# AI-Application-and-Integration-Lab/RDPN6D

Measured on AMD Instinct MI355X. Metric: RGB-D crops/sec (fwd+PnP) at 256x256, higher is better.
Workload: dtype f32

## Files before the change

### include/rdpn6d.h

```cpp
#ifndef RDPN6D_H
#define RDPN6D_H

#ifdef __cplusplus
extern "C" {
#endif

#define RDPN6D_OK 0
#define RDPN6D_EINVAL -1
#define RDPN6D_EHIP -2
#define RDPN6D_ENOMEM -3

const char* rdpn6d_last_error(void);
int rdpn6d_version(void);
int rdpn6d_device_count(void);

void farthest_point_sampling(float* pts, int* idxs, int pn, int sn);
void farthest_point_sampling_init_center(float* pts, int* idxs, int pn, int sn);
int rdpn6d_fps_host(const float* pts, int* idxs, int pn, int sn, int start);
int rdpn6d_fps_device(const float* d_pts, const int* d_offsets, int nobj, int max_pn, int sn, int start,
                      int* d_idxs, float* d_mindist, void* stream);
long long rdpn6d_fps_workspace_bytes(int nobj);
int rdpn6d_fps_device_ws(const float* d_pts, const int* d_offsets, int nobj, int max_pn, int sn, int start, int* d_idxs,
                         float* d_mindist, void* workspace, long long workspace_bytes, void* stream);

// ... 9 lines not shown
    int in_cs, in_co;
    int Ho, Wo;
    int stride;
    int ntaps;
    int dy[9], dx[9];
    int N, Npad;
    int OH, OW;
    int osy, osx, ooy, oox;
    int out_cs, out_co;
    int res_cs, res_co;
    int act;
    float slope;
} rdpn6d_conv_desc;
int rdpn6d_conv2d_f32(const rdpn6d_conv_desc* d, void* stream);
long long rdpn6d_conv_splitk_ws_floats(const rdpn6d_conv_desc* d, int ksplit);
int rdpn6d_conv2d_splitk_f32(const rdpn6d_conv_desc* d, int ksplit, float* workspace, void* stream);
int rdpn6d_conv_tile_for(const rdpn6d_conv_desc* d, int* bm, int* bn);
void rdpn6d_conv_force_tile(int bm, int bn);
void rdpn6d_conv_set_tap_inner(int v);

int rdpn6d_conv2d_bf16(const rdpn6d_conv_desc* d, int out_f32, void* stream);
int rdpn6d_conv2d_splitk_bf16(const rdpn6d_conv_desc* d, int out_f32, int ksplit, float* workspace, void* stream);
int rdpn6d_conv2d_bf16_bnstats(const rdpn6d_conv_desc* d, double* stats, int stats_row0, int* stats_rows, void* stream);
int rdpn6d_conv2d_bf16_bnbwd(const rdpn6d_conv_desc* d, const void* bn_x, int bn_cs, int bn_co, const float* mean, const float* invstd,
                             const float* gamma, const float* beta, double* partial, int* rows, void* stream);
int rdpn6d_bn_relu_backward_apply_bf16(const void* x, int xcs, int xco, const void* dy, int dcs, int dco, const float* mean,
                                       const float* invstd, const float* gamma, const float* beta, float* dgamma, float* dbeta, void* dx,
                                       int xgcs, int xgco, long long M, int C, const double* partial, int S, void* stream);
int rdpn6d_conv2d_bf16_bnbwd_y(const rdpn6d_conv_desc* d, const void* bn_x, int bn_cs, int bn_co, const void* bn_y, int y_cs, int y_co,
                               const float* mean, const float* invstd, double* partial, int* rows, void* stream);
int rdpn6d_bn_backward_apply_bf16(const void* x, int xcs, int xco, const void* dy, int dcs, int dco, const void* y, int ycs, int yco,
                                  const float* mean, const float* invstd, const float* gamma, float* dgamma, float* dbeta, void* dx,
                                  int xgcs, int xgco, void* dres, int rcs, int rco, long long M, int C, const double* partial, int S,
                                  void* stream);
void rdpn6d_conv_bf16_force_tile(int bm, int bn);
void rdpn6d_conv_bf16_force_stages(int nst);
int rdpn6d_conv_bf16_tile_for(const rdpn6d_conv_desc* d, int* bm, int* bn);
int rdpn6d_conv_bf16_uses_pingpong(const rdpn6d_conv_desc* d, int out_f32);
int rdpn6d_split_bf16x3(const float* x, long long n, void* planes, long long plane_elems, void* stream);
int rdpn6d_conv_bf16x3_eligible(const rdpn6d_conv_desc* d);
int rdpn6d_conv_bf16x3_kernel_for(const rdpn6d_conv_desc* d);
int rdpn6d_conv2d_bf16x3(const rdpn6d_conv_desc* d, long long x_plane_elems, long long w_plane_elems, void* y_planes,
                         long long y_plane_elems, void* stream);
int rdpn6d_conv2d_bf16x3_ex(const rdpn6d_conv_desc* d, long long x_plane_elems, long long w_plane_elems, void* y_planes,
                            long long y_plane_elems, const void* res_planes, long long res_plane_elems, void* stream);
int rdpn6d_split_h2(const float* x, int src_cs, int src_co, int C, void* dst, long long npix, int* overflow_flag, void* stream);
int rdpn6d_conv_h2_kernel_for(const rdpn6d_conv_desc* d);
int rdpn6d_conv2d_h2(const rdpn6d_conv_desc* d, void* y_h2, const void* res_h2, int* overflow_flag, void* stream);
int rdpn6d_conv2d_h2_cb(const rdpn6d_conv_desc* d, void* y_h2, const void* res_h2, int* overflow_flag, const float* crop_bias,
                        void* stream);
long long rdpn6d_conv_h2_workspace_bytes(const rdpn6d_conv_desc* d);
void rdpn6d_conv_h2_set_clock_probe(unsigned long long* buf);
void rdpn6d_conv_h2_set_wfrag(int mode);
int rdpn6d_conv_h2_colmax_ok(const rdpn6d_conv_desc* d, int rows_per_group);
int rdpn6d_conv2d_h2_colmax(const rdpn6d_conv_desc* d, unsigned long long* keys, int rows_per_group, int* overflow_flag, void* stream);
int rdpn6d_h2_colmax_decode(unsigned long long* keys, int groups, int N, int Npad, void* out_h2, void* stream);
int rdpn6d_conv_h2_wfrag_wanted(const rdpn6d_conv_desc* d);
int rdpn6d_h2_weight_frag(const void* w_h2, int Npad, int ntaps, int cchunks, void* w_frag, void* stream);
int rdpn6d_conv2d_h2_wf(const rdpn6d_conv_desc* d, void* y_h2, const void* res_h2, int* overflow_flag, const void* w_frag, void* stream);
int rdpn6d_conv2d_h2_ws(const rdpn6d_conv_desc* d, void* y_h2, const void* res_h2, int* overflow_flag, const float* crop_bias,
                        void* workspace, long long workspace_bytes, void* stream);
int rdpn6d_conv_h2_fuse1x1_ok(const rdpn6d_conv_desc* d);
int rdpn6d_conv2d_h2_fuse1x1(const rdpn6d_conv_desc* d, const void* res_h2, int* overflow_flag, const float* crop_bias,
                             const void* w1_h2, const float* scale1, const float* bias1, float* out, int out_cs, int n_out,
                             void* stream);
int rdpn6d_upsample_bilinear_h2(const void* x, int B, int H, int W, int C, int factor, void* y, int* overflow_flag, void* stream);
int rdpn6d_upsample_bilinear_h2_ex(const void* x, int B, int H, int W, int C, int factor, void* y, int out_cs, int out_co, int relu,
                                   int* overflow_flag, void* stream);
int rdpn6d_xyz_subsample_h2(const float* x, int B, int xc, int R, int step, void* y, int out_cs, int out_co, int* overflow_flag,
                            void* stream);
int rdpn6d_global_max_concat_h2(void* buf, int B, int HW, int C, int cs, void* stream);
int rdpn6d_global_max_h2(const void* x_h2, int B, int HW, int C, int cs, void* gmax_h2, void* stream);
int rdpn6d_convt3x3s2_const_bias_f32(const float* V, const float* scale, int B, int F, float* out , void* stream);
int rdpn6d_stem_pool_h2(const float* x, int B, int xc, int R, const void* w_h2, const float* scale, const float* shift, void* y,
                        int* overflow_flag, void* stream);
int rdpn6d_stem_pool_h2_ex(const float* x, int B, int xc, int R, const void* w_h2, const float* scale, const float* shift, void* y,
                           int out_fmt, int* overflow_flag, void* stream);
int rdpn6d_stem_pack_h2(const float* w_oihw, void* w_h2, float* inv_scale, void* stream);
void rdpn6d_conv_bf16_force_chunk(int row_bytes);
int rdpn6d_stem_conv7x7_bf16(const float* x, int B, int xc, int R, const float* w, const float* scale,
                             const float* shift, void* y, void* stream);
int rdpn6d_maxpool3x3s2_bf16(const void* x, int B, int H, int W, int C, void* y, void* stream);
int rdpn6d_upsample_bilinear_bf16(const void* x, int B, int H, int W, int C, int factor, void* y, void* stream);
int rdpn6d_xyz_subsample_bf16(const float* x, int B, int xc, int R, int step, void* y, int out_cs, int out_co,
                              void* stream);
int rdpn6d_global_max_concat_bf16(void* buf, int B, int HW, int C, int cs, void* stream);
int rdpn6d_cast_f32_bf16(const float* src, int src_cs, int src_co, int C, void* dst, int dst_cs, long long npix,
                         void* stream);

int rdpn6d_stem_conv7x7_f32(const float* x, int B, int xc, int R, const float* w, const float* scale,
                            const float* shift, float* y, void* stream);
int rdpn6d_maxpool3x3s2_f32(const float* x, int B, int H, int W, int C, float* y, void* stream);
int rdpn6d_upsample_bilinear_f32(const float* x, int B, int H, int W, int C, int factor, float* y, void* stream);
int rdpn6d_xyz_subsample_f32(const float* x, int B, int xc, int R, int step, float* y, int out_cs, int out_co,
                             void* stream);
int rdpn6d_global_max_concat_f32(float* buf, int B, int HW, int C, int cs, void* stream);
int rdpn6d_groupnorm_relu_f32(float* x, int B, int HW, int C, int G, const float* gamma, const float* beta,
                              void* stream);
int rdpn6d_groupnorm_relu_h2(const float* x, int B, int HW, int C, int G, const float* gamma, const float* beta, void* y_h2,
                             int* overflow_flag, void* stream);

int rdpn6d_dense_glue_f32(const float* head, int head_cs, const float* coord2d, const float* fps, int B, int HW,
                          int K, int mask_attention, float* minmax_scratch, float* out_nchw, float* pnp_in,
                          int pnp_cs, int* argmax_out, void* stream);
int rdpn6d_dense_glue_h2(const float* head, int head_cs, const float* coord2d, const float* fps, int B, int HW, int K,
                         int mask_attention, float* minmax_scratch, float* out_nchw, void* pnp_in_h2, int pnp_cs,
// ... 260 lines not shown
```

### rdpn6d_amd/_lib.py

```python
import ctypes
import os

HERE = os.path.dirname(os.path.abspath(__file__))
LIB_PATH = os.environ.get("RDPN6D_LIB") or os.path.join(HERE, "librdpn6d_hip.so")

_ll = ctypes.c_longlong
c_float_p = ctypes.c_void_p
c_int_p = ctypes.c_void_p
_vp, _i, _f, _u = ctypes.c_void_p, ctypes.c_int, ctypes.c_float, ctypes.c_uint


class ConvDesc(ctypes.Structure):

    _fields_ = [
        ("x", _vp), ("w", _vp), ("scale", _vp), ("shift", _vp), ("res", _vp), ("y", _vp),
        ("B", _i), ("H", _i), ("W", _i), ("Cin", _i), ("in_cs", _i), ("in_co", _i), ("Ho", _i), ("Wo", _i),
        ("stride", _i), ("ntaps", _i), ("dy", _i * 9), ("dx", _i * 9), ("N", _i), ("Npad", _i), ("OH", _i), ("OW", _i),
        ("osy", _i), ("osx", _i), ("ooy", _i), ("oox", _i), ("out_cs", _i), ("out_co", _i), ("res_cs", _i),
        ("res_co", _i), ("act", _i), ("slope", _f),
    ]


SIGNATURES = {
    "rdpn6d_last_error": (ctypes.c_char_p, []),
# ... 83 lines not shown
    "rdpn6d_dense_glue_backward_f32": (_i, [_vp, _i, _vp, _vp, _vp, _vp, _i, _i, _i, _i, _i, _vp, _vp, _vp, _vp]),
    "rdpn6d_dense_losses_mt_f32": (_i, [_vp, _i, _vp, _vp, _vp, _vp, _i, _i, _i, _f, _f, _f, _i, _vp, _vp, _vp, _vp]),
    "rdpn6d_dense_glue_backward_mt_f32": (_i, [_vp, _i, _vp, _vp, _vp, _vp, _i, _i, _i, _i, _i, _i, _vp, _vp, _vp, _vp]),
    "rdpn6d_pose_train_f32": (_i, [_vp, _i, _vp, _vp, _vp, _vp, _vp, _vp, _vp, _vp, _i, _i, _i, _f, _i, _f, _f, _vp, _vp, _vp,
                                   _vp, _vp, _vp]),
    "rdpn6d_pose_train_sym_f32": (_i, [_vp, _i, _vp, _vp, _vp, _vp, _vp, _vp, _vp, _vp, _i, _i, _i, _f, _i, _f, _f, _vp, _vp, _i,
                                       _vp, _vp, _vp, _vp, _vp, _vp, _vp]),
    "rdpn6d_ranger_step_f32": (_i, [_vp, _vp, _vp, _vp, _vp, _vp, _i, _vp, _vp, _i, _vp, _f, _f, _f, _f, _f, _i, _i, _f, _vp]),
    "rdpn6d_ranger_step_scaled_f32": (_i, [_vp, _vp, _vp, _vp, _vp, _vp, _i, _vp, _vp, _i, _vp, _f, _f, _f, _f, _f, _i, _i, _f, _f, _vp, _vp]),
    "rdpn6d_grad_nonfinite_f32": (_i, [_vp, _ll, _vp, _vp]),
    "rdpn6d_region_targets_f32": (_i, [_vp, _vp, _vp, _vp, _i, _i, _i, _vp, _vp, _vp]),
    "rdpn6d_pose_errors_f64": (_i, [_vp, _vp, _vp, _i, _i, _i, _vp, _vp, _vp]),
    "rdpn6d_crop_builder_f32": (_i, [_vp, _vp, _i, _i, _i, _vp, _vp, _vp, _vp, _vp, _i, _i, _vp, _vp, _vp]),
    "rdpn6d_act_backward_f32": (_i, [_vp, _vp, _ll, _f, _vp]),
    "rdpn6d_transpose_rc_f32": (_i, [_vp, _i, _i, _i, _vp, _vp]),
    "rdpn6d_train_vis_scalars_f32": (_i, [_vp, _vp, _vp, _vp, _vp, _i, _vp, _i, _vp, _vp]),
    "rdpn6d_rgb_to_nhwc4_f32": (_i, [_vp, _i, _i, _i, _vp, _vp]),
    "rdpn6d_stem_im2col_f32": (_i, [_vp, _i, _i, _i, _vp, _vp]),
    "rdpn6d_stem_rowpatch_f32": (_i, [_vp, _i, _i, _i, _vp, _vp]),
    "rdpn6d_stem_conv7x7_raw_bf16": (_i, [_vp, _i, _i, _i, _vp, _vp, _vp]),
    "rdpn6d_bn_train_stats_bf16": (_i, [_vp, _ll, _i, _i, _i, _f, _f, _vp, _vp, _vp, _vp, _vp, _vp]),
    "rdpn6d_bn_apply_bf16": (_i, [_vp, _i, _i, _vp, _vp, _vp, _vp, _vp, _i, _i, _vp, _i, _i, _ll, _i, _i, _vp]),
    "rdpn6d_bn_backward_bf16": (_i, [_vp, _i, _i, _vp, _i, _i, _vp, _i, _i, _vp, _vp, _vp, _vp, _vp, _vp, _i, _i, _vp, _i, _i,
                                     _ll, _i, _i, _vp, _vp]),
    "rdpn6d_bn_relu_backward_bf16": (_i, [_vp, _i, _i, _vp, _i, _i, _vp, _vp, _vp, _vp, _vp, _vp, _vp, _i, _i, _ll, _i, _vp, _vp]),
    "rdpn6d_channel_sum_bf16": (_i, [_vp, _ll, _i, _i, _i, _vp, _i, _vp, _vp]),
    "rdpn6d_maxpool3x3s2_backward_bf16": (_i, [_vp, _vp, _i, _i, _i, _i, _vp, _vp]),
    "rdpn6d_upsample_bilinear_backward_bf16": (_i, [_vp, _i, _i, _i, _i, _i, _vp, _vp]),
    "rdpn6d_global_max_concat_backward_bf16": (_i, [_vp, _vp, _i, _i, _i, _i, _vp, _vp]),
    "rdpn6d_stem_im2col_bf16": (_i, [_vp, _i, _i, _i, _vp, _vp]),
    "rdpn6d_stem_rowpatch_bf16": (_i, [_vp, _i, _i, _i, _vp, _vp]),
    "rdpn6d_repack_f32": (_i, [_vp, _vp, _vp, _i, _vp]),
    "rdpn6d_split_h2": (_i, [_vp, _i, _i, _i, _vp, _ll, _vp, _vp]),
    "rdpn6d_conv_h2_kernel_for": (_i, [_vp]),
    "rdpn6d_conv2d_h2": (_i, [_vp, _vp, _vp, _vp, _vp]),
    "rdpn6d_upsample_bilinear_h2": (_i, [_vp, _i, _i, _i, _i, _i, _vp, _vp, _vp]),
    "rdpn6d_xyz_subsample_h2": (_i, [_vp, _i, _i, _i, _i, _vp, _i, _i, _vp, _vp]),
    "rdpn6d_stem_pool_h2": (_i, [_vp, _i, _i, _i, _vp, _vp, _vp, _vp, _vp, _vp]),
    "rdpn6d_stem_pool_h2_ex": (_i, [_vp, _i, _i, _i, _vp, _vp, _vp, _vp, _i, _vp, _vp]),
    "rdpn6d_stem_pack_h2": (_i, [_vp, _vp, _vp, _vp]),
    "rdpn6d_global_max_concat_h2": (_i, [_vp, _i, _i, _i, _i, _vp]),
    "rdpn6d_upsample_bilinear_h2_ex": (_i, [_vp, _i, _i, _i, _i, _i, _vp, _i, _i, _i, _vp, _vp]),
    "rdpn6d_global_max_h2": (_i, [_vp, _i, _i, _i, _i, _vp, _vp]),
    "rdpn6d_convt3x3s2_const_bias_f32": (_i, [_vp, _vp, _i, _i, _vp, _vp]),
    "rdpn6d_conv2d_h2_cb": (_i, [_vp, _vp, _vp, _vp, _vp, _vp]),
    "rdpn6d_conv2d_h2_ws": (_i, [_vp, _vp, _vp, _vp, _vp, _vp, ctypes.c_longlong, _vp]),
    "rdpn6d_conv_h2_fuse1x1_ok": (_i, [ctypes.POINTER(ConvDesc)]),
    "rdpn6d_conv2d_h2_fuse1x1": (_i, [ctypes.POINTER(ConvDesc), _vp, _vp, _vp, _vp, _vp, _vp, _vp, _i, _i, _vp]),
    "rdpn6d_conv_h2_workspace_bytes": (ctypes.c_longlong, [_vp]),
    "rdpn6d_conv_h2_colmax_ok": (_i, [ctypes.POINTER(ConvDesc), _i]),
    "rdpn6d_conv2d_h2_colmax": (_i, [ctypes.POINTER(ConvDesc), _vp, _i, _vp, _vp]),
    "rdpn6d_h2_colmax_decode": (_i, [_vp, _i, _i, _i, _vp, _vp]),
    "rdpn6d_conv_h2_set_wfrag": (None, [_i]),
    "rdpn6d_conv_h2_set_clock_probe": (None, [_vp]),
    "rdpn6d_conv_h2_wfrag_wanted": (_i, [ctypes.POINTER(ConvDesc)]),
    "rdpn6d_h2_weight_frag": (_i, [_vp, _i, _i, _i, _vp, _vp]),
    "rdpn6d_conv2d_h2_wf": (_i, [ctypes.POINTER(ConvDesc), _vp, _vp, _vp, _vp, _vp]),
    "rdpn6d_ransac_pnp_f32": (_i, [_vp, _vp, _vp, _vp, _vp, _i, _i, _f, _i, _f, ctypes.c_uint, _i, _f, _vp, _vp, _vp, _vp, _vp]),
    "rdpn6d_ransac_pnp_ex": (_i, [_vp, _vp, _vp, _vp, _vp, _i, _i, _f, _i, _f, ctypes.c_uint, _i, _f, _i, _vp, _vp, _vp, _vp, _vp]),
    "rdpn6d_ransac_pnp_workspace_bytes": (_ll, [_i]),
    "rdpn6d_ransac_pnp_ws": (_i, [_vp, _vp, _vp, _vp, _vp, _i, _i, _f, _i, _f, ctypes.c_uint, _i, _f, _i, _vp, _vp, _vp, _vp, _vp, _ll, _vp]),
    "rdpn6d_select_correspondences_f32": (_i, [_vp, _i, _vp, _i, _i, _i, _vp, _vp, _i, _i, _i, _i, _f, _vp, _vp, _vp, _vp, _vp, _vp]),
    "rdpn6d_select_correspondences_mt_f32": (_i, [_vp, _i, _vp, _i, _i, _i, _vp, _vp, _i, _i, _i, _i, _f, _i, _vp, _vp, _vp, _vp, _vp, _vp]),
}

for _k in [k for k in list(SIGNATURES) if "_bf16" in k and "bf16x3" not in k]:
    SIGNATURES[_k.replace("_bf16", "_fp16")] = SIGNATURES[_k]
SIGNATURES["rdpn6d_repack_fp16"] = SIGNATURES["rdpn6d_repack_f32"]

_lib = None


def load():
    global _lib
    if _lib is None:
        if not os.path.exists(LIB_PATH):
            raise RuntimeError(
                f"{LIB_PATH} is missing: build the HIP extension first (python -m rdpn6d_amd.build). "
                "rdpn6d_amd has no CPU fallback."
            )
        import torch

        if torch.cuda.device_count() > 0:
            torch.cuda.init()
        lib = ctypes.CDLL(LIB_PATH)
        for name, (res, args) in SIGNATURES.items():
            fn = getattr(lib, name)
            fn.restype = res
            fn.argtypes = args
        _lib = lib
    return _lib


def check(rc, what=""):
    if rc != 0:
        msg = load().rdpn6d_last_error()
        raise RuntimeError(f"rdpn6d HIP call failed ({what}, rc={rc}): {msg.decode() if msg else '?'}")
```

### rdpn6d_amd/csrc/conv_igemm_h2.hip

```cpp
#include "conv_h2_common.h"

#include <cstdio>
#include <cstdlib>

#ifdef RDPN6D_PROBE
__device__ unsigned long long* g_h2_probe = nullptr;
extern "C" int rdpn6d_debug_h2_probe(void* buf)
{
    RD_CHECK_HIP(hipMemcpyToSymbol(HIP_SYMBOL(g_h2_probe), &buf, sizeof(buf)));
    return RDPN6D_OK;
}
#endif

namespace {

constexpr int HT_BYTES = 16384;
constexpr int LDS_8PH = 2 * 4 * HT_BYTES;
constexpr int LDS_8PH_FUSED = 8 * (32 * 72 * 4 + 32 * 272);
static_assert(LDS_8PH_FUSED >= LDS_8PH && LDS_8PH_FUSED <= 160 * 1024, "LDS");

template <bool FUSE, bool CMAX>
__device__ __forceinline__ void conv_h2_8ph_body(const ConvH2Args& ax)
{
    extern __shared__ __attribute__((aligned(1024))) unsigned char smem[];
// ... 845 lines not shown
        *reinterpret_cast<f16x8*>(pp) = hi;
        *reinterpret_cast<f16x8*>(pp + 32) = lo;
    }
    if (over && overflow_flag) *overflow_flag = 1;
}

bool h2_common_ok(const rdpn6d_conv_desc* d)
{
    return d->Cin % 32 == 0 && d->in_cs % 32 == 0 && d->in_co % 32 == 0 && d->out_cs % 8 == 0 && d->out_co % 8 == 0 && d->N % 8 == 0 &&
           d->Npad % 64 == 0 && (!d->res || (d->res_cs % 4 == 0 && d->res_co % 4 == 0));
}
bool h2_big_ok(const rdpn6d_conv_desc* d)
{
    const int nk = d->ntaps * (d->Cin / 32);
    return h2_common_ok(d) && d->Npad % 256 == 0 && d->N == d->Npad && nk >= 2 && (nk & 1) == 0;
}
bool h2_big_pays(const rdpn6d_conv_desc* d, long long M)
{
    const long long tiles = (long long)rd_cdiv(M, 256) * (d->Npad / 256);
    const long long rounds = (tiles + 255) / 256;
    return tiles >= 160 && (double)tiles >= 0.62 * 256.0 * (double)rounds;
}
void h2_pick_tile(const rdpn6d_conv_desc* d, long long M, int* pbm, int* pbn)
{
    int bn = (d->Npad % 128 == 0) ? 128 : 64;
    int bm = 128;
    if ((long long)rd_cdiv(M, 128) * (d->Npad / bn) < 512) bm = 64;
    if (bm == 64 && bn == 128 && (long long)rd_cdiv(M, 64) * (d->Npad / 128) < 512) bn = 64;
    if (const char* f = getenv("RDPN6D_H2_TILE")) {
        int fbm = 0, fbn = 0;
        if (sscanf(f, "%d,%d", &fbm, &fbn) == 2 && (fbm == 64 || fbm == 128) && (fbn == 64 || fbn == 128) && d->Npad % fbn == 0) {
            bm = fbm;
            bn = fbn;
        }
    }
    *pbm = bm;
    *pbn = bn;
}

}

extern "C" int rdpn6d_split_h2(const float* x, int src_cs, int src_co, int C, void* dst, long long npix, int* overflow_flag, void* stream)
{
    RD_REQUIRE(x && dst && npix > 0 && C > 0 && C % 32 == 0 && src_cs % 4 == 0 && src_co % 4 == 0 && src_co + C <= src_cs, "h2 split: C % 32, aligned slice");
    const long long blocks = (npix * (C / 8) + 255) / 256;
    hipLaunchKernelGGL(split_h2_kernel, dim3((unsigned)(blocks > 16384 ? 16384 : blocks)), dim3(256), 0, (hipStream_t)stream, x, src_cs,
                       src_co, C, (_Float16*)dst, npix, overflow_flag);
    RD_LAUNCH_CHECK();
    return RDPN6D_OK;
}

int conv_h2_launch_pp(ConvH2Args& ax, int shape, hipStream_t s);

static int h2_pp_plan(const rdpn6d_conv_desc* d, long long M, int* pbm, int* pbn)
{
    static const int on = getenv("RDPN6D_H2_PP") ? atoi(getenv("RDPN6D_H2_PP")) : 1;
    static const int force = getenv("RDPN6D_H2_PP_SHAPE") ? atoi(getenv("RDPN6D_H2_PP_SHAPE")) : -1;
    if (!on || d->Npad % 128 != 0 || d->ntaps * (d->Cin / 32) < 8) return -1;
    int shape = 0;
    if ((long long)rd_cdiv(M, 256) * (d->Npad / 128) >= 224 && (long long)rd_cdiv(M, 128) * (d->Npad / 128) > 288) shape = 2;
    if (force == 0 || force == 2) shape = force;
    const int bm = shape == 0 ? 128 : 256;
    if ((long long)rd_cdiv(M, bm) * (d->Npad / 128) < 224) return -1;
    *pbm = bm;
    *pbn = 128;
    return shape;
}

static int h2_tile_ksplit(const rdpn6d_conv_desc* d, long long M, int bm, int bn)
{
    static const int off = getenv("RDPN6D_H2_NO_SPLITK") ? 1 : 0;
    const long long tiles = (long long)rd_cdiv(M, bm) * (d->Npad / bn);
    static const int tmax = getenv("RDPN6D_H2_SPLIT_TILES") ? atoi(getenv("RDPN6D_H2_SPLIT_TILES")) : 128;
    if (off || tiles >= tmax) return 0;
    const int nk = d->ntaps * (d->Cin / 32);
    int best = 0;
    for (int sl = 2; sl <= 32; sl *= 2)
        if (tiles * sl <= 512 && nk % sl == 0 && nk / sl >= 4) best = sl;
    return best;
}

static int g_h2_wfrag_mode = getenv("RDPN6D_H2_BFG") ? atoi(getenv("RDPN6D_H2_BFG")) : 0;
extern "C" void rdpn6d_conv_h2_set_wfrag(int mode) { g_h2_wfrag_mode = mode; }
static unsigned long long* g_h2_clk_probe = nullptr;
extern "C" void rdpn6d_conv_h2_set_clock_probe(unsigned long long* buf) { g_h2_clk_probe = buf; }
static bool h2_wfrag_shape_ok(int shape)
{
    const int mode = g_h2_wfrag_mode;
    return mode >= 1 && (shape == 0 || (mode >= 2 && shape == 2));
}

extern "C" int rdpn6d_conv_h2_kernel_for(const rdpn6d_conv_desc* d)
{
    if (!d || !h2_common_ok(d)) return 0;
    const long long M = (long long)d->B * d->Ho * d->Wo;
    return (h2_big_ok(d) && h2_big_pays(d, M)) ? 2 : 1;
}

extern "C" int rdpn6d_conv2d_h2_cb(const rdpn6d_conv_desc* d, void* y_h2, const void* res_h2, int* overflow_flag, const float* crop_bias,
                                   void* stream);
extern "C" int rdpn6d_conv2d_h2(const rdpn6d_conv_desc* d, void* y_h2, const void* res_h2, int* overflow_flag, void* stream)
{
    return rdpn6d_conv2d_h2_cb(d, y_h2, res_h2, overflow_flag, nullptr, stream);
}

extern "C" long long rdpn6d_conv_h2_workspace_bytes(const rdpn6d_conv_desc* d)
{
    if (!d || rdpn6d_conv_h2_kernel_for(d) != 1) return 0;
    const long long M = (long long)d->B * d->Ho * d->Wo;
    int bm, bn;
    if (h2_pp_plan(d, M, &bm, &bn) >= 0) return 0;
    h2_pick_tile(d, M, &bm, &bn);
    return (long long)h2_tile_ksplit(d, M, bm, bn) * rd_cdiv(M, bm) * bm * d->Npad * 4;
}

extern "C" int rdpn6d_conv2d_h2_ws(const rdpn6d_conv_desc* d, void* y_h2, const void* res_h2, int* overflow_flag, const float* crop_bias,
// ... 228 lines not shown
```

### rdpn6d_amd/csrc/conv_igemm_h2_pp.hip

```cpp
#include "conv_h2_common.h"

#include <cstdio>
#include <cstdlib>

#ifdef RDPN6D_PROBE
__device__ unsigned long long* g_h2pp_probe = nullptr;
extern "C" int rdpn6d_debug_h2pp_probe(void* buf)
{
    RD_CHECK_HIP(hipMemcpyToSymbol(HIP_SYMBOL(g_h2pp_probe), &buf, sizeof(buf)));
    return RDPN6D_OK;
}
#define PP_T(i) const unsigned long long pt##i = __builtin_readcyclecounter(); __builtin_amdgcn_sched_barrier(0)
#define PP_ACC(j, a, b) pp_sum[j] += pt##b - pt##a
#else
#define PP_T(i)
#define PP_ACC(j, a, b)
#endif

namespace {

template <int BM, int BN, int WM, int WN, int NST, int PM, bool BFG = false>
__global__ __launch_bounds__(512) void conv_h2_pp_kernel(const ConvH2Args ax)
{
    constexpr int RB = 128, RPP = 8, NW = 8;
    constexpr int WTM = BM / WM, WTN = BN / WN, TM = WTM / 32, TN = WTN / 32;
    constexpr int AG = BM / RPP / NW, BG = BFG ? 0 : BN / RPP / NW;
    constexpr int NB = BFG ? 4 * TN : 0;
    constexpr int P = AG + BG, PL = P - PM, D = NST - 1;
    constexpr int Q = P + NB;
    static_assert(WM * WN == NW && WM == 2 && TM >= 1 && TN >= 1 && AG >= 1 && (BFG || BG >= 1), "wave grid / tile");
    static_assert(PM >= 0 && PM <= 2 && PL >= 1 && D >= 2, "pieces in the MFMA part; at least three stages");
    extern __shared__ __attribute__((aligned(1024))) unsigned char smem[];
    unsigned char* As = smem;
    unsigned char* Bs = smem + NST * BM * RB;
#ifdef RDPN6D_PROBE
    const unsigned long long pp_start = __builtin_readcyclecounter();
    unsigned long long pp_e[6] = {0, 0, 0, 0, 0, 0};
#endif

    const ConvBArgs& a = ax.b;
    const rdpn6d_conv_desc& d = a.d;
    const int nblk = a.mtiles * a.ntiles;
    const int bid = blockIdx.x;
    const int q8 = nblk >> 3, r8 = nblk & 7, xcd = bid & 7, kk = bid >> 3;
    const int logical = (xcd < r8 ? xcd * (q8 + 1) : r8 * (q8 + 1) + (xcd - r8) * q8) + kk;
    const int nt = logical % a.ntiles;
    const int mt = logical / a.ntiles;
    const long long m0 = (long long)mt * BM;
    const int n0 = nt * BN;

    const int tid = threadIdx.x;
    const int lane = tid & 63;
    const int wave = __builtin_amdgcn_readfirstlane(tid >> 6);
    const int grp = wave >> 2, wq = wave & 3;
    const int wm = grp, wn = wq;

    const int prow = lane >> 3, pslot = lane & 7;
    const unsigned px_bytes = (unsigned)d.in_cs * 4u;
    unsigned a_base[AG], a_mask[AG];
#pragma unroll
    for (int i = 0; i < AG; ++i) {
        const int row = (wave + NW * i) * RPP + prow;
        const long long m = m0 + row;
        const bool ok = m < a.M;
        const int mm = ok ? (int)m : 0;
        const int b = mm / a.HoWo;
        const int rem = mm - b * a.HoWo;
        const int oy = rem / d.Wo;
        const int ox = rem - oy * d.Wo;
        const int iy = oy * d.stride, ix = ox * d.stride;
        const int lslot = pslot ^ ((row >> 1) & 7);
        a_base[i] = (unsigned)((b * d.H + iy) * d.W + ix) * px_bytes + (unsigned)d.in_co * 4u + (unsigned)lslot * 16u;
        unsigned mask = 0;
        for (int t = 0; t < d.ntaps; ++t) {
            const int dy = (int)((a.dy_pack >> (4 * t)) & 15ull) - 8, dx = (int)((a.dx_pack >> (4 * t)) & 15ull) - 8;
            mask |= (ok && (unsigned)(iy + dy) < (unsigned)d.H && (unsigned)(ix + dx) < (unsigned)d.W) ? (1u << t) : 0u;
        }
        a_mask[i] = mask;
    }
    unsigned w_off[BG > 0 ? BG : 1];
#pragma unroll
    for (int i = 0; i < BG; ++i) {
        const int row = (wave + NW * i) * RPP + prow;
        const int lslot = pslot ^ ((row >> 1) & 7);
// ... 30 lines not shown
        if constexpr (first + 2 < last) stage_piece(ic<first + 2>{}, st);
        if constexpr (first + 3 < last) stage_piece(ic<first + 3>{}, st);
        if constexpr (first + 4 < last) stage_piece(ic<first + 4>{}, st);
        if constexpr (first + 5 < last) stage_piece(ic<first + 5>{}, st);
        if constexpr (first + 6 < last) stage_piece(ic<first + 6>{}, st);
        if constexpr (first + 7 < last) stage_piece(ic<first + 7>{}, st);
        static_assert(last - first <= 8, "pieces per wave and chunk");
    };

    constexpr int CS = WTN + 8, LPR = WTN / 8, RPI = 64 / LPR, NRR = 32 / RPI;
    const int frow = lane & 31;
    const int nb = n0 + wn * WTN;
    const int rrow = lane / LPR, c8 = (lane % LPR) * 8;
    const long long mbase = m0 + wm * WTM;
    f16x8 rh[TM][NRR], rl[TM][NRR];
    long long pixs[TM][NRR];
    const bool res_pre = ax.res_h2 != nullptr && d.res == nullptr;
#pragma unroll
    for (int i = 0; i < TM; ++i)
#pragma unroll
        for (int rr = 0; rr < NRR; ++rr) {
            const long long mrow = mbase + i * 32 + rr * RPI + rrow;
            const bool ok = mrow < a.M && nb + c8 < d.N;
            pixs[i][rr] = ok ? h2_pixel_of(a, mrow) : -1;
            if (res_pre && ok) {
                const int c = d.res_co + nb + c8;
                const _Float16* rp = reinterpret_cast<const _Float16*>(ax.res_h2) + pixs[i][rr] * (2 * d.res_cs) + (c >> 5) * 64 + (c & 31);
                rh[i][rr] = *reinterpret_cast<const f16x8*>(rp);
                rl[i][rr] = *reinterpret_cast<const f16x8*>(rp + 32);
            } else {
                rh[i][rr] = f16x8{};
                rl[i][rr] = f16x8{};
            }
        }
    float scj[TN], shj[TN];
#pragma unroll
    for (int j = 0; j < TN; ++j) {
        const int n = nb + j * 32 + frow;
        scj[j] = d.scale ? d.scale[n] : 1.f;
        shj[j] = d.shift ? d.shift[n] : 0.f;
    }

    const int nk = a.nk;
    int ld_cc = 0, ld_tap = 0, ld_idx = 0;
    auto next_chunk = [&]() {
        ++ld_idx;
        ++ld_tap;
        const int wrap = ld_tap == d.ntaps ? 1 : 0;
        ld_tap = wrap ? 0 : ld_tap;
        ld_cc += wrap;
    };

    const int half = lane >> 5;
    u32x4 fa[TM][4], fb[BFG ? 3 * TN : TN][4];
    const unsigned wf_lane = (unsigned)lane * 16u;
    const unsigned wf_n32 = (unsigned)(n0 + wn * WTN) / 32u;
    auto load_bfrags = [&](auto slotc, const int tap, const int cc, const bool valid) {
        constexpr int slot = decltype(slotc)::value;
        if constexpr (BFG) {
#pragma unroll
            for (int jn = 0; jn < TN; ++jn) {
                const unsigned base = (((wf_n32 + (unsigned)jn) * (unsigned)d.ntaps + (unsigned)tap) * (unsigned)a.cchunks + (unsigned)cc) * 4096u;
                const unsigned so = valid ? base : 0xFFFFF000u;
#pragma unroll
                for (int j = 0; j < 4; ++j)
                    fb[slot * TN + jn][j] = __builtin_bit_cast(u32x4, __builtin_amdgcn_raw_buffer_load_b128(wsrc, (int)wf_lane, (int)(so + j * 1024u), 0));
            }
        }
    };
    auto read_frags = [&](const int st) {
#pragma unroll
        for (int i = 0; i < TM; ++i) {
            const int R = wm * WTM + i * 32 + frow;
            const int sw = (R >> 1) & 7;
            const unsigned char* q = As + ((st * BM) + R) * RB;
#pragma unroll
            for (int j = 0; j < 4; ++j) fa[i][j] = *reinterpret_cast<const u32x4*>(q + (((2 * j + half) ^ sw) << 4));
        }
        if constexpr (!BFG) {
#pragma unroll
            for (int jn = 0; jn < TN; ++jn) {
                const int R = wn * WTN + jn * 32 + frow;
                const int sw = (R >> 1) & 7;
                const unsigned char* q = Bs + ((st * BN) + R) * RB;
#pragma unroll
                for (int j = 0; j < 4; ++j) fb[jn][j] = *reinterpret_cast<const u32x4*>(q + (((2 * j + half) ^ sw) << 4));
            }
        }
    };

    f32x16 acc[TM][TN];
#pragma unroll
    for (int i = 0; i < TM; ++i)
#pragma unroll
        for (int j = 0; j < TN; ++j)
#pragma unroll
            for (int e = 0; e < 16; ++e) acc[i][j][e] = 0.f;

    auto mma_group = [&](auto prc, auto slotc) {
        constexpr int pr = decltype(prc)::value, slot = decltype(slotc)::value;
        H2_PAIRS;
#pragma unroll
        for (int i = 0; i < TM; ++i)
#pragma unroll
            for (int jn = 0; jn < TN; ++jn) acc[i][jn] = h2_mfma(fa[i][H2_PA[pr]], fb[slot * TN + jn][H2_PB[pr]], acc[i][jn]);
    };

    int lb_cc = 0, lb_tap = 0, lb_idx = 0;
    auto next_b = [&]() {
        ++lb_idx;
        ++lb_tap;
        const int wrap = lb_tap == d.ntaps ? 1 : 0;
        lb_tap = wrap ? 0 : lb_tap;
        lb_cc += wrap;
    };
    static_assert(!BFG || D <= 3, "BFG: the counted waits below assume the weight stream (2 chunks ahead) is not behind the DMA ring");

    auto pro_step = [&](auto cc_) {
        constexpr int c = decltype(cc_)::value;
        if constexpr (c < D) {
            stage_addr(ld_tap, ld_cc, ld_idx < nk);
            stage_pieces(ic<0>{}, ic<PL>{}, c);
            if constexpr (BFG && c - D + 2 >= 0) {
                load_bfrags(ic<c - D + 2>{}, lb_tap, lb_cc, lb_idx < nk);
                next_b();
            }
            stage_pieces(ic<PL>{}, ic<P>{}, c);
            next_chunk();
        }
    };
    pro_step(ic<0>{});
    pro_step(ic<1>{});
    pro_step(ic<2>{});
    pro_step(ic<3>{});
    static_assert(D <= 4, "prologue steps");
    stage_addr(ld_tap, ld_cc, ld_idx < nk);
    asm volatile("s_waitcnt vmcnt(%0)" ::"n"((D - 1) * Q) : "memory");
    __builtin_amdgcn_s_barrier();
    asm volatile("" ::: "memory");
    if (grp == 1) __builtin_amdgcn_s_barrier();

    int st_rd = 0, st_wr = D;
#ifdef RDPN6D_PROBE
    unsigned long long pp_sum[6] = {0, 0, 0, 0, 0, 0};
    const unsigned long long pp_t0 = __builtin_readcyclecounter();
#endif
    constexpr int N1a = (D - 2) * Q + PL + NB, N1 = (BFG && N1a > 2 * Q) ? 2 * Q : N1a, N3 = (D - 1) * Q;
    static_assert(N1 <= 63 && N3 <= 63, "vmcnt is a 6-bit counter");
    auto step = [&](auto slotc) {
        constexpr int slot = decltype(slotc)::value;
        __builtin_amdgcn_sched_barrier(0);
        PP_T(0);
        read_frags(st_rd);
        __builtin_amdgcn_sched_barrier(0);
        stage_pieces(ic<0>{}, ic<PL>{}, st_wr);
        if constexpr (BFG) {
            load_bfrags(ic<(slot + 2) % 3>{}, lb_tap, lb_cc, lb_idx < nk);
            next_b();
        }
        __builtin_amdgcn_sched_barrier(0);
        PP_T(1);
        asm volatile("s_waitcnt vmcnt(%0) lgkmcnt(0)" ::"n"(N1) : "memory");
        PP_T(2);
        __builtin_amdgcn_s_barrier();
        asm volatile("" ::: "memory");
        __builtin_amdgcn_sched_barrier(0);
        PP_T(3);
        __builtin_amdgcn_s_setprio(1);
        mma_group(ic<0>{}, slotc);
        mma_group(ic<1>{}, slotc);
        __builtin_amdgcn_sched_barrier(0);
        if constexpr (PM >= 1) stage_piece(ic<PL>{}, st_wr);
        __builtin_amdgcn_sched_barrier(0);
        mma_group(ic<2>{}, slotc);
        mma_group(ic<3>{}, slotc);
        __builtin_amdgcn_sched_barrier(0);
        if constexpr (PM >= 2) stage_piece(ic<PL + 1>{}, st_wr);
        __builtin_amdgcn_sched_barrier(0);
        next_chunk();
        stage_addr(ld_tap, ld_cc, ld_idx < nk);
        mma_group(ic<4>{}, slotc);
        mma_group(ic<5>{}, slotc);
        __builtin_amdgcn_s_setprio(0);
        __builtin_amdgcn_sched_barrier(0);
        PP_T(4);
        st_rd = st_rd == NST - 1 ? 0 : st_rd + 1;
        st_wr = st_wr == NST - 1 ? 0 : st_wr + 1;
        asm volatile("s_waitcnt vmcnt(%0)" ::"n"(N3) : "memory");
        PP_T(5);
        __builtin_amdgcn_s_barrier();
        asm volatile("" ::: "memory");
        PP_T(6);
        PP_ACC(0, 0, 1);
        PP_ACC(1, 1, 2);
        PP_ACC(2, 2, 3);
        PP_ACC(3, 3, 4);
        PP_ACC(4, 4, 5);
        PP_ACC(5, 5, 6);
    };
    if constexpr (BFG) {
        int k = 0;
        for (; k + 3 <= nk; k += 3) {
            step(ic<0>{});
            step(ic<1>{});
            step(ic<2>{});
        }
        if (k < nk) step(ic<0>{});
        if (k + 1 < nk) step(ic<1>{});
    } else {
        for (int k = 0; k < nk; ++k) step(ic<0>{});
    }
#ifdef RDPN6D_PROBE
    const unsigned long long pp_loop_end = __builtin_readcyclecounter();
#endif
    asm volatile("s_waitcnt vmcnt(0)" ::: "memory");
    if (grp == 0) __builtin_amdgcn_s_barrier();
#ifdef RDPN6D_PROBE
    pp_e[0] = __builtin_readcyclecounter();
#endif

    {
        const int hi = lane >> 5;
        __builtin_amdgcn_s_barrier();
        asm volatile("" ::: "memory");
#ifdef RDPN6D_PROBE
        pp_e[1] = __builtin_readcyclecounter();
#endif
        float* cst = reinterpret_cast<float*>(smem) + wave * (32 * CS);
#pragma unroll
        for (int i = 0; i < TM; ++i) {
#pragma unroll
            for (int j = 0; j < TN; ++j)
#pragma unroll
                for (int e = 0; e < 16; ++e)
                    cst[((e & 3) + 8 * (e >> 2) + 4 * hi) * CS + j * 32 + frow] = acc[i][j][e] * scj[j] + shj[j];
#pragma unroll
            for (int rr = 0; rr < NRR; ++rr) {
                const int row = rr * RPI + rrow;
                if (pixs[i][rr] >= 0) {
                    const f32x4 lo = *reinterpret_cast<const f32x4*>(cst + row * CS + c8);
                    const f32x4 hi4 = *reinterpret_cast<const f32x4*>(cst + row * CS + c8 + 4);
                    float v[8] = {lo[0], lo[1], lo[2], lo[3], hi4[0], hi4[1], hi4[2], hi4[3]};
                    if (res_pre) h2_finish_row8_t<true>(ax, v, pixs[i][rr], nb + c8, rh[i][rr], rl[i][rr]);
                    else h2_finish_row8_t<false>(ax, v, pixs[i][rr], nb + c8, rh[i][rr], rl[i][rr]);
                }
            }
        }
    }
#ifdef RDPN6D_PROBE
    pp_e[2] = __builtin_readcyclecounter();
    asm volatile("s_waitcnt vmcnt(0)" ::: "memory");
    pp_e[3] = __builtin_readcyclecounter();
    if (g_h2pp_probe && lane == 0) {
        unsigned long long* o = g_h2pp_probe + ((size_t)blockIdx.x * 8 + wave) * 16;
        for (int i = 0; i < 6; ++i) o[i] = pp_sum[i];
        o[6] = pp_loop_end - pp_t0;
        o[7] = (unsigned long long)nk;
        o[8] = pp_t0 - pp_start;
        o[9] = pp_e[0] - pp_loop_end;
        o[10] = pp_e[1] - pp_e[0];
        o[11] = pp_e[2] - pp_e[1];
        o[12] = pp_e[3] - pp_e[2];
    }
#endif
}

template <int BM, int BN, int WM, int WN, int NST, int PM, bool BFG = false>
int launch_pp(const ConvH2Args& ax, hipStream_t s)
{
    constexpr int lds_stage = NST * (BM + (BFG ? 0 : BN)) * 128;
    constexpr int lds_epi = 8 * 32 * (BN / WN + 8) * 4;
    constexpr int lds = lds_stage > lds_epi ? lds_stage : lds_epi;
    static_assert(lds <= 160 * 1024, "LDS");
    auto kern = conv_h2_pp_kernel<BM, BN, WM, WN, NST, PM, BFG>;
    RD_LDS_OPT_IN(kern, lds);
    hipLaunchKernelGGL(kern, dim3((unsigned)(ax.b.mtiles * ax.b.ntiles)), dim3(512), lds, s, ax);
    return RDPN6D_OK;
}

}

int conv_h2_launch_pp(ConvH2Args& ax, int shape, hipStream_t s)
{
    static const int pm = getenv("RDPN6D_H2_PP_PM") ? atoi(getenv("RDPN6D_H2_PP_PM")) : 2;
    if (ax.w_frag) {
        static const int bpm = getenv("RDPN6D_H2_BFG_PM") ? atoi(getenv("RDPN6D_H2_BFG_PM")) : 1;
        if (shape == 0) return bpm == 0 ? launch_pp<128, 128, 2, 4, 4, 0, true>(ax, s) : launch_pp<128, 128, 2, 4, 4, 1, true>(ax, s);
        if (shape == 2) return bpm == 0 ? launch_pp<256, 128, 2, 4, 4, 0, true>(ax, s) : bpm == 1 ? launch_pp<256, 128, 2, 4, 4, 1, true>(ax, s) : launch_pp<256, 128, 2, 4, 4, 2, true>(ax, s);
    }
    if (shape == 0) return pm == 0 ? launch_pp<128, 128, 2, 4, 4, 0>(ax, s) : pm == 1 ? launch_pp<128, 128, 2, 4, 4, 1>(ax, s) : launch_pp<128, 128, 2, 4, 4, 2>(ax, s);
    if (shape == 2) return pm == 0 ? launch_pp<256, 128, 2, 4, 3, 0>(ax, s) : pm == 1 ? launch_pp<256, 128, 2, 4, 3, 1>(ax, s) : launch_pp<256, 128, 2, 4, 3, 2>(ax, s);
    rdpn6d_set_error("conv_h2_launch_pp: unknown tile shape %d", shape);
    return RDPN6D_EINVAL;
}
```

Before: 9486.

## Add pipelined BM=64 pingpong conv variant for small-tile-count h2 convolutions

Adds a PIPE form of the pingpong implicit-GEMM kernel. It double-buffers fragment registers and interleaves the LDS fragment reads for the next k-step between the MFMA groups of the current one, with a 6-stage, 64-row tile configuration. The planner now sends convolutions that have too few 128/256-row tiles to this BM=64 kernel instead of the fallback path, which should raise occupancy and overlap on smaller layers. A runtime policy setter controls the minimum tile count and can disable the form. The cost is higher register pressure from the two fragment sets, plus deeper vmcnt bookkeeping that could stall or reduce occupancy.

```diff
diff --git a/include/rdpn6d.h b/include/rdpn6d.h
--- a/include/rdpn6d.h
+++ b/include/rdpn6d.h
@@ -85,6 +85,7 @@
 long long rdpn6d_conv_h2_workspace_bytes(const rdpn6d_conv_desc* d);
 void rdpn6d_conv_h2_set_clock_probe(unsigned long long* buf);
 void rdpn6d_conv_h2_set_wfrag(int mode);
+void rdpn6d_conv_h2_set_pp_policy(int min_tiles, int form);
 int rdpn6d_conv_h2_colmax_ok(const rdpn6d_conv_desc* d, int rows_per_group);
 int rdpn6d_conv2d_h2_colmax(const rdpn6d_conv_desc* d, unsigned long long* keys, int rows_per_group, int* overflow_flag, void* stream);
 int rdpn6d_h2_colmax_decode(unsigned long long* keys, int groups, int N, int Npad, void* out_h2, void* stream);
diff --git a/rdpn6d_amd/_lib.py b/rdpn6d_amd/_lib.py
--- a/rdpn6d_amd/_lib.py
+++ b/rdpn6d_amd/_lib.py
@@ -159,6 +159,7 @@
     "rdpn6d_conv2d_h2_colmax": (_i, [ctypes.POINTER(ConvDesc), _vp, _i, _vp, _vp]),
     "rdpn6d_h2_colmax_decode": (_i, [_vp, _i, _i, _i, _vp, _vp]),
     "rdpn6d_conv_h2_set_wfrag": (None, [_i]),
+    "rdpn6d_conv_h2_set_pp_policy": (None, [_i, _i]),
     "rdpn6d_conv_h2_set_clock_probe": (None, [_vp]),
     "rdpn6d_conv_h2_wfrag_wanted": (_i, [ctypes.POINTER(ConvDesc)]),
     "rdpn6d_h2_weight_frag": (_i, [_vp, _i, _i, _i, _vp, _vp]),
diff --git a/rdpn6d_amd/csrc/conv_igemm_h2.hip b/rdpn6d_amd/csrc/conv_igemm_h2.hip
--- a/rdpn6d_amd/csrc/conv_igemm_h2.hip
+++ b/rdpn6d_amd/csrc/conv_igemm_h2.hip
@@ -921,6 +921,14 @@
 
 int conv_h2_launch_pp(ConvH2Args& ax, int shape, hipStream_t s);
 
+static int g_h2_pp_min_tiles = 0, g_h2_pp_form = -1;
+extern "C" void rdpn6d_conv_h2_set_pp_policy(int min_tiles, int form)
+{
+    g_h2_pp_min_tiles = min_tiles;
+    g_h2_pp_form = form;
+}
+static bool h2_pp_pipe() { return g_h2_pp_form != 0; }
+
 static int h2_pp_plan(const rdpn6d_conv_desc* d, long long M, int* pbm, int* pbn)
 {
     static const int on = getenv("RDPN6D_H2_PP") ? atoi(getenv("RDPN6D_H2_PP")) : 1;
@@ -929,8 +937,13 @@
     int shape = 0;
     if ((long long)rd_cdiv(M, 256) * (d->Npad / 128) >= 224 && (long long)rd_cdiv(M, 128) * (d->Npad / 128) > 288) shape = 2;
     if (force == 0 || force == 2) shape = force;
-    const int bm = shape == 0 ? 128 : 256;
-    if ((long long)rd_cdiv(M, bm) * (d->Npad / 128) < 224) return -1;
+    int bm = shape == 0 ? 128 : 256;
+    const int min_tiles = g_h2_pp_min_tiles > 0 ? g_h2_pp_min_tiles : 224;
+    if ((long long)rd_cdiv(M, bm) * (d->Npad / 128) < min_tiles) {
+        if (!h2_pp_pipe() || force >= 0 || (long long)rd_cdiv(M, 64) * (d->Npad / 128) < min_tiles) return -1;
+        bm = 64;
+        shape = 3;
+    }
     *pbm = bm;
     *pbn = 128;
     return shape;
diff --git a/rdpn6d_amd/csrc/conv_igemm_h2_pp.hip b/rdpn6d_amd/csrc/conv_igemm_h2_pp.hip
--- a/rdpn6d_amd/csrc/conv_igemm_h2_pp.hip
+++ b/rdpn6d_amd/csrc/conv_igemm_h2_pp.hip
@@ -19,17 +19,18 @@
 
 namespace {
 
-template <int BM, int BN, int WM, int WN, int NST, int PM, bool BFG = false>
+template <int BM, int BN, int WM, int WN, int NST, int PM, bool BFG = false, bool PIPE = false>
 __global__ __launch_bounds__(512) void conv_h2_pp_kernel(const ConvH2Args ax)
 {
     constexpr int RB = 128, RPP = 8, NW = 8;
     constexpr int WTM = BM / WM, WTN = BN / WN, TM = WTM / 32, TN = WTN / 32;
     constexpr int AG = BM / RPP / NW, BG = BFG ? 0 : BN / RPP / NW;
     constexpr int NB = BFG ? 4 * TN : 0;
-    constexpr int P = AG + BG, PL = P - PM, D = NST - 1;
+    constexpr int P = AG + BG, PL = P - PM, D = PIPE ? NST : NST - 1;
     constexpr int Q = P + NB;
     static_assert(WM * WN == NW && WM == 2 && TM >= 1 && TN >= 1 && AG >= 1 && (BFG || BG >= 1), "wave grid / tile");
     static_assert(PM >= 0 && PM <= 2 && PL >= 1 && D >= 2, "pieces in the MFMA part; at least three stages");
+    static_assert(!(PIPE && BFG) && (!PIPE || (PM == 0 && TM + TN <= 3)), "the pipelined form: weights through LDS, two fragment sets in registers");
     extern __shared__ __attribute__((aligned(1024))) unsigned char smem[];
     unsigned char* As = smem;
     unsigned char* Bs = smem + NST * BM * RB;
@@ -166,7 +167,7 @@
     };
 
     const int half = lane >> 5;
-    u32x4 fa[TM][4], fb[BFG ? 3 * TN : TN][4];
+    u32x4 fa[PIPE ? 2 * TM : TM][4], fb[BFG ? 3 * TN : PIPE ? 2 * TN : TN][4];
     const unsigned wf_lane = (unsigned)lane * 16u;
     const unsigned wf_n32 = (unsigned)(n0 + wn * WTN) / 32u;
     auto load_bfrags = [&](auto slotc, const int tap, const int cc, const bool valid) {
@@ -182,25 +183,30 @@
             }
         }
     };
-    auto read_frags = [&](const int st) {
-#pragma unroll
-        for (int i = 0; i < TM; ++i) {
-            const int R = wm * WTM + i * 32 + frow;
+    auto read_tile = [&](auto tc, auto setc, const int st) {
+        constexpr int t = decltype(tc)::value, set = decltype(setc)::value;
+        if constexpr (t < TM) {
+            const int R = wm * WTM + t * 32 + frow;
             const int sw = (R >> 1) & 7;
             const unsigned char* q = As + ((st * BM) + R) * RB;
 #pragma unroll
-            for (int j = 0; j < 4; ++j) fa[i][j] = *reinterpret_cast<const u32x4*>(q + (((2 * j + half) ^ sw) << 4));
-        }
-        if constexpr (!BFG) {
-#pragma unroll
-            for (int jn = 0; jn < TN; ++jn) {
-                const int R = wn * WTN + jn * 32 + frow;
-                const int sw = (R >> 1) & 7;
-                const unsigned char* q = Bs + ((st * BN) + R) * RB;
-#pragma unroll
-                for (int j = 0; j < 4; ++j) fb[jn][j] = *reinterpret_cast<const u32x4*>(q + (((2 * j + half) ^ sw) << 4));
-            }
-        }
+            for (int j = 0; j < 4; ++j) fa[set * TM + t][j] = *reinterpret_cast<const u32x4*>(q + (((2 * j + half) ^ sw) << 4));
+        } else if constexpr (!BFG && t < TM + TN) {
+            constexpr int jn = t - TM;
+            const int R = wn * WTN + jn * 32 + frow;
+            const int sw = (R >> 1) & 7;
+            const unsigned char* q = Bs + ((st * BN) + R) * RB;
+#pragma unroll
+            for (int j = 0; j < 4; ++j) fb[set * TN + jn][j] = *reinterpret_cast<const u32x4*>(q + (((2 * j + half) ^ sw) << 4));
+        }
+    };
+    auto read_frags = [&](auto setc, const int st) {
+        read_tile(ic<0>{}, setc, st);
+        read_tile(ic<1>{}, setc, st);
+        read_tile(ic<2>{}, setc, st);
+        read_tile(ic<3>{}, setc, st);
+        read_tile(ic<4>{}, setc, st);
+        static_assert(TM + TN <= 5, "fragment tiles per wave");
     };
 
     f32x16 acc[TM][TN];
@@ -212,12 +218,12 @@
             for (int e = 0; e < 16; ++e) acc[i][j][e] = 0.f;
 
     auto mma_group = [&](auto prc, auto slotc) {
-        constexpr int pr = decltype(prc)::value, slot = decltype(slotc)::value;
+        constexpr int pr = decltype(prc)::value, slot = decltype(slotc)::value, aset = PIPE ? slot : 0;
         H2_PAIRS;
 #pragma unroll
         for (int i = 0; i < TM; ++i)
 #pragma unroll
-            for (int jn = 0; jn < TN; ++jn) acc[i][jn] = h2_mfma(fa[i][H2_PA[pr]], fb[slot * TN + jn][H2_PB[pr]], acc[i][jn]);
+            for (int jn = 0; jn < TN; ++jn) acc[i][jn] = h2_mfma(fa[aset * TM + i][H2_PA[pr]], fb[slot * TN + jn][H2_PB[pr]], acc[i][jn]);
     };
 
     int lb_cc = 0, lb_tap = 0, lb_idx = 0;
@@ -247,14 +253,26 @@
     pro_step(ic<1>{});
     pro_step(ic<2>{});
     pro_step(ic<3>{});
-    static_assert(D <= 4, "prologue steps");
+    pro_step(ic<4>{});
+    pro_step(ic<5>{});
+    static_assert(D <= 6, "prologue steps");
     stage_addr(ld_tap, ld_cc, ld_idx < nk);
-    asm volatile("s_waitcnt vmcnt(%0)" ::"n"((D - 1) * Q) : "memory");
-    __builtin_amdgcn_s_barrier();
-    asm volatile("" ::: "memory");
-    if (grp == 1) __builtin_amdgcn_s_barrier();
-
-    int st_rd = 0, st_wr = D;
+    if constexpr (PIPE) {
+        asm volatile("s_waitcnt vmcnt(%0)" ::"n"((D - 2) * Q) : "memory");
+        __builtin_amdgcn_s_barrier();
+        asm volatile("" ::: "memory");
+        read_frags(ic<0>{}, 0);
+        asm volatile("s_waitcnt lgkmcnt(0)" ::: "memory");
+        __builtin_amdgcn_s_barrier();
+        asm volatile("" ::: "memory");
+    } else {
+        asm volatile("s_waitcnt vmcnt(%0)" ::"n"((D - 1) * Q) : "memory");
+        __builtin_amdgcn_s_barrier();
+        asm volatile("" ::: "memory");
+        if (grp == 1) __builtin_amdgcn_s_barrier();
+    }
+
+    int st_rd = PIPE ? 1 : 0, st_wr = D % NST;
 #ifdef RDPN6D_PROBE
     unsigned long long pp_sum[6] = {0, 0, 0, 0, 0, 0};
     const unsigned long long pp_t0 = __builtin_readcyclecounter();
@@ -265,7 +283,7 @@
         constexpr int slot = decltype(slotc)::value;
         __builtin_amdgcn_sched_barrier(0);
         PP_T(0);
-        read_frags(st_rd);
+        read_frags(ic<0>{}, st_rd);
         __builtin_amdgcn_sched_barrier(0);
         stage_pieces(ic<0>{}, ic<PL>{}, st_wr);
         if constexpr (BFG) {
@@ -312,7 +330,66 @@
         PP_ACC(4, 4, 5);
         PP_ACC(5, 5, 6);
     };
-    if constexpr (BFG) {
+    constexpr int NP = (D - 2) * P;
+    static_assert(!PIPE || NP <= 63, "vmcnt is a 6-bit counter");
+    auto pstep = [&](auto curc) {
+        constexpr int cur = decltype(curc)::value;
+        using nxt = ic<cur ^ 1>;
+        constexpr int RT = TM + TN;
+        constexpr int PH = (P + 1) / 2;
+        auto gap = [&](auto gc, auto vc) {
+            constexpr int g = decltype(gc)::value, v = decltype(vc)::value;
+            constexpr int r = v == 0 ? g : g - 2;
+            constexpr int h = v == 0 ? g - RT : g;
+            __builtin_amdgcn_sched_barrier(0);
+            if constexpr (h == 0) stage_pieces(ic<0>{}, ic<PH>{}, st_wr);
+            if constexpr (h == 1) {
+                stage_pieces(ic<PH>{}, ic<P>{}, st_wr);
+                next_chunk();
+                stage_addr(ld_tap, ld_cc, ld_idx < nk);
+            }
+            if constexpr (r >= 0 && r < RT) read_tile(ic<(r >= 0 && r < RT) ? r : 0>{}, nxt{}, st_rd);
+            __builtin_amdgcn_sched_barrier(0);
+        };
+        static_assert(RT + 2 <= 5, "five gaps");
+        auto body = [&](auto vc) {
+            mma_group(ic<0>{}, curc);
+            gap(ic<0>{}, vc);
+            mma_group(ic<1>{}, curc);
+            gap(ic<1>{}, vc);
+            mma_group(ic<2>{}, curc);
+            gap(ic<2>{}, vc);
+            mma_group(ic<3>{}, curc);
+            gap(ic<3>{}, vc);
+            mma_group(ic<4>{}, curc);
+            gap(ic<4>{}, vc);
+            mma_group(ic<5>{}, curc);
+        };
+        __builtin_amdgcn_sched_barrier(0);
+        PP_T(0);
+        if (grp == 0) body(ic<0>{});
+        else body(ic<1>{});
+        __builtin_amdgcn_sched_barrier(0);
+        PP_T(1);
+        st_rd = st_rd == NST - 1 ? 0 : st_rd + 1;
+        st_wr = st_wr == NST - 1 ? 0 : st_wr + 1;
+        asm volatile("s_waitcnt vmcnt(%0) lgkmcnt(0)" ::"n"(NP) : "memory");
+        PP_T(2);
+        __builtin_amdgcn_s_barrier();
+        asm volatile("" ::: "memory");
+        PP_T(3);
+        PP_ACC(3, 0, 1);
+        PP_ACC(4, 1, 2);
+        PP_ACC(5, 2, 3);
+    };
+    if constexpr (PIPE) {
+        int k = 0;
+        for (; k + 2 <= nk; k += 2) {
+            pstep(ic<0>{});
+            pstep(ic<1>{});
+        }
+        if (k < nk) pstep(ic<0>{});
+    } else if constexpr (BFG) {
         int k = 0;
         for (; k + 3 <= nk; k += 3) {
             step(ic<0>{});
@@ -328,7 +405,7 @@
     const unsigned long long pp_loop_end = __builtin_readcyclecounter();
 #endif
     asm volatile("s_waitcnt vmcnt(0)" ::: "memory");
-    if (grp == 0) __builtin_amdgcn_s_barrier();
+    if (!PIPE && grp == 0) __builtin_amdgcn_s_barrier();
 #ifdef RDPN6D_PROBE
     pp_e[0] = __builtin_readcyclecounter();
 #endif
@@ -379,14 +456,14 @@
 #endif
 }
 
-template <int BM, int BN, int WM, int WN, int NST, int PM, bool BFG = false>
+template <int BM, int BN, int WM, int WN, int NST, int PM, bool BFG = false, bool PIPE = false>
 int launch_pp(const ConvH2Args& ax, hipStream_t s)
 {
     constexpr int lds_stage = NST * (BM + (BFG ? 0 : BN)) * 128;
     constexpr int lds_epi = 8 * 32 * (BN / WN + 8) * 4;
     constexpr int lds = lds_stage > lds_epi ? lds_stage : lds_epi;
     static_assert(lds <= 160 * 1024, "LDS");
-    auto kern = conv_h2_pp_kernel<BM, BN, WM, WN, NST, PM, BFG>;
+    auto kern = conv_h2_pp_kernel<BM, BN, WM, WN, NST, PM, BFG, PIPE>;
     RD_LDS_OPT_IN(kern, lds);
     hipLaunchKernelGGL(kern, dim3((unsigned)(ax.b.mtiles * ax.b.ntiles)), dim3(512), lds, s, ax);
     return RDPN6D_OK;
@@ -396,6 +473,7 @@
 
 int conv_h2_launch_pp(ConvH2Args& ax, int shape, hipStream_t s)
 {
+    if (shape == 3) return launch_pp<64, 128, 2, 4, 6, 0, false, true>(ax, s);
     static const int pm = getenv("RDPN6D_H2_PP_PM") ? atoi(getenv("RDPN6D_H2_PP_PM")) : 2;
     if (ax.w_frag) {
         static const int bpm = getenv("RDPN6D_H2_BFG_PM") ? atoi(getenv("RDPN6D_H2_BFG_PM")) : 1;
```

After: 9518 (median of 6 runs). No clear change (+0.3%).
